# kuwt/model_matching

Measured on AMD Instinct MI355X. Metric: candidate poses verified/sec, higher is better.
Workload: dtype f32; 1 GPU; Cm: synthetic 20000-pt scene vs 5000-pt model, 65536 candidate transforms per step per GPU, eps=5mm; scene_points=20000, model_points=5000

## Files before the change

### model_matching_amd/csrc/lcp.hip

```cpp
#include <stdlib.h>
#include <string.h>

#include <cstring>


#include <algorithm>
#include <utility>

#include "kdtree.h"
#include "normal_cone.h"
#include "octant_lists.h"
#include "prims.h"
#include "stocs_ctx.h"

namespace stocs {

struct LcpArgs {
    const float4* mpos;
    const float4* mnrm;
    const int32_t* mperm;
    int M;
    const int32_t* top;
    const uint4* cells;
    const uint4* flat;
    const float4* list;
    const float4* snrmw;
    const int32_t* cand_trial;
    size_t snrmw_stride;
    const float* chunk_r;
    float ox, oy, oz, inv_h, inv_h4, h;
    int nx, ny, nz, nbx, nby;
    float sq_eps, dot_lo, eps;
    float bound_margin;
    int has_nearest;
    const int32_t* order;
    int xcd_blocks;
    unsigned long long* best;
    uint32_t id_offset;
    const float4* patch;
    const float4* sub;
    const float* dist;
    float gox, goy, goz, g, inv_g, cap;
    int gnx, gny, gnz;
#ifdef STOCS_TOOLS_BUILD
    int ablate;
#endif
};
#ifdef STOCS_TOOLS_BUILD
#define STOCS_ABLATE(a, bit) (((a).ablate & (bit)) != 0)
#else
#define STOCS_ABLATE(a, bit) false
#endif

__device__ __forceinline__ int lcp_candidate(const LcpArgs& a, int n, int w, int wpb = 4) {
    int blk = blockIdx.x;
    if (a.xcd_blocks == 1) {
        const int nb = gridDim.x, per = nb >> 3, rem = nb & 7, xcd = blk & 7;
        blk = xcd * per + (xcd < rem ? xcd : rem) + (blk >> 3);
    } else if (a.xcd_blocks > 1) {
        const int C = a.xcd_blocks, nb = gridDim.x, full = (nb / (8 * C)) * (8 * C);
        if (blk < full) {
            const int xcd = blk & 7, j = blk >> 3;
            blk = ((j / C) * 8 + xcd) * C + (j % C);
        }
    }
    const int slot = __builtin_amdgcn_readfirstlane(blk * wpb + w);
    if (slot >= n) return -1;
    return a.order ? __builtin_amdgcn_readfirstlane(a.order[slot]) : slot;
}


__device__ __forceinline__ const float4* lcp_weights_of(const LcpArgs& a, int cand) {
    if (!a.cand_trial) return a.snrmw;
    const int t = __builtin_amdgcn_readfirstlane(a.cand_trial[cand < 0 ? 0 : cand]);
    return (const float4*)((const char*)a.snrmw + (size_t)t * a.snrmw_stride);
}

#define DPP_QUAD_XOR1 0xB1
#define DPP_QUAD_XOR2 0x4E
#define DPP_HALF_MIRROR 0x141

__device__ __forceinline__ void lcp_add(unsigned long long& acc, float w) {
    if (w > 0.0f) acc += (unsigned long long)(w * 4294967296.0f);
}
__device__ __forceinline__ unsigned long long lcp_wave_sum(unsigned long long acc) {
    for (int off = 32; off > 0; off >>= 1) acc += __shfl_xor(acc, off, 64);
    return acc;
}
__device__ __forceinline__ float lcp_finish(unsigned long long total, int M) {
    return (float)((double)total * (1.0 / 4294967296.0) / (double)M);
}
__device__ __forceinline__ void lcp_store(const LcpArgs& a, float* __restrict__ out, int cand, unsigned long long total) {
    const float s = lcp_finish(total, a.M);
    out[cand] = s;
    if (a.best && s > 0.0f)
        atomicMax(a.best, best_key(s, a.id_offset + (uint32_t)cand));
}

template <bool IDX>
__device__ __forceinline__ void take_if_better(float d, int ei, float& gd, int& gi) {
    if (IDX) { if (d <= gd) { gd = d; gi = ei; } }
    else { if (d < gd || (d == gd && ei > gi)) { gd = d; gi = ei; } }
}

template <bool DETAIL, bool IDX = true>
__global__ __launch_bounds__(256) void lcp_kernel(LcpArgs a, const float* __restrict__ T16, float* __restrict__ out,
                                                  int n, int32_t* __restrict__ hit_out, uint8_t* __restrict__ cnt_out) {
    const int lane = threadIdx.x & 63;
    const int cand = lcp_candidate(a, n, threadIdx.x >> 6);
    if (cand < 0) return;
    const float* T = T16 + (size_t)cand * 16;
    const float4* __restrict__ snrmw = lcp_weights_of(a, cand);
    const float t0 = T[0], t1 = T[1], t2 = T[2], t4 = T[4], t5 = T[5], t6 = T[6], t8 = T[8], t9 = T[9], t10 = T[10],
                t12 = T[12], t13 = T[13], t14 = T[14];
    unsigned long long acc = 0ull;
    for (int i = lane; i < a.M; i += 64) {
        const float4 p = a.mpos[i];
        const float qx = ((t0 * p.x + t4 * p.y) + t8 * p.z) + t12;
        const float qy = ((t1 * p.x + t5 * p.y) + t9 * p.z) + t13;
        const float qz = ((t2 * p.x + t6 * p.y) + t10 * p.z) + t14;
        const float fx = floorf((qx - a.ox) * a.inv_h);
        const float fy = floorf((qy - a.oy) * a.inv_h);
        const float fz = floorf((qz - a.oz) * a.inv_h);
        int best = -1;
        if (fx >= 0.0f && fy >= 0.0f && fz >= 0.0f && fx < (float)a.nx && fy < (float)a.ny && fz < (float)a.nz) {
            const int cx = (int)fx, cy = (int)fy, cz = (int)fz;
            const int brick = a.top[((cz >> 3) * a.nby + (cy >> 3)) * a.nbx + (cx >> 3)];
            if (brick >= 0) {
                const uint4 cw = a.cells[(size_t)brick * 512 + (((cz & 7) << 6) | ((cy & 7) << 3) | (cx & 7))];
                float bd = a.sq_eps;
                const uint32_t cn = cw.y & STOCS_CONE_COUNT_MASK;
                for (uint32_t k = 0; k < cn; ++k) {
                    const float4 s = a.list[cw.x + k];
                    const float dx = qx - s.x, dy = qy - s.y, dz = qz - s.z;
                    const float d = dx * dx + (dy * dy + dz * dz);
                    take_if_better<IDX>(d, __float_as_int(s.w), bd, best);
                }
            }
        }
        bool counted = false;
        if (best >= 0) {
            const float4 nm = a.mnrm[i];
            const float nx = t0 * nm.x + (t4 * nm.y + t8 * nm.z);
            const float ny = t1 * nm.x + (t5 * nm.y + t9 * nm.z);
            const float nz = t2 * nm.x + (t6 * nm.y + t10 * nm.z);
            const float4 sn = snrmw[best];
            const float d = sn.x * nx + (sn.y * ny + sn.z * nz);
            counted = (d >= a.dot_lo) && (d <= 1.0f);
            if (counted) lcp_add(acc, sn.w);
        }
        if (DETAIL) {
            const int orig = a.mperm[i];
            hit_out[(size_t)cand * a.M + orig] = best;
            cnt_out[(size_t)cand * a.M + orig] = counted ? 1 : 0;
        }
    }
    acc = lcp_wave_sum(acc);
    if (lane == 0) lcp_store(a, out, cand, acc);
}

template <int CTRL>
__device__ __forceinline__ float dpp_f32(float v) {
    return __int_as_float(__builtin_amdgcn_update_dpp(0, __float_as_int(v), CTRL, 0xF, 0xF, true));
}
template <int CTRL>
__device__ __forceinline__ int dpp_i32(int v) {
    return __builtin_amdgcn_update_dpp(0, v, CTRL, 0xF, 0xF, true);
}

template <int GL>
__device__ __forceinline__ float group_min_nonneg(float v) {
    uint32_t u = __float_as_uint(v);
    if (GL >= 2) u = min(u, (uint32_t)__builtin_amdgcn_update_dpp((int)u, (int)u, DPP_QUAD_XOR1, 0xF, 0xF, false));
    if (GL >= 4) u = min(u, (uint32_t)__builtin_amdgcn_update_dpp((int)u, (int)u, DPP_QUAD_XOR2, 0xF, 0xF, false));
    if (GL == 8) u = min(u, (uint32_t)__builtin_amdgcn_update_dpp((int)u, (int)u, DPP_HALF_MIRROR, 0xF, 0xF, false));
    return __uint_as_float(u);
}

constexpr int lcp_waves_per_block(bool detail, bool split) { return (split || detail) ? 4 : 1; }

template <bool DETAIL, bool SPLIT>
__global__ __launch_bounds__(64 * lcp_waves_per_block(DETAIL, SPLIT)) void lcp_coop_kernel(LcpArgs a, const float* __restrict__ T16, float* __restrict__ out,
                                                       int n, int32_t* __restrict__ hit_out, uint8_t* __restrict__ cnt_out) {
    static_assert(!(DETAIL && SPLIT), "the detail form is not split");
    constexpr int WPB = lcp_waves_per_block(DETAIL, SPLIT);
    constexpr int UNR = 2;
    __shared__ float4 qt[WPB][64];
    __shared__ uint32_t qn[WPB][64];
    __shared__ uint32_t hl[WPB][64];
    __shared__ float rd[WPB][64];
    __shared__ int ri[WPB][64];
    __shared__ float qd[WPB][64];
    __shared__ unsigned long long part[WPB];
    const int lane = threadIdx.x & 63;
    const int sub = lane & 7, grp = lane >> 3;
    const int w = threadIdx.x >> 6;
    const int cand = SPLIT ? lcp_candidate(a, n, 0, 1) : lcp_candidate(a, n, w, WPB);
    if (cand < 0) return;
    const int first = SPLIT ? 64 * w : 0, stride = SPLIT ? 64 * WPB : 64;
    const float4* __restrict__ snrmw = lcp_weights_of(a, cand);
    const float* T = T16 + (size_t)cand * 16;
    const float t0 = T[0], t1 = T[1], t2 = T[2], t4 = T[4], t5 = T[5], t6 = T[6], t8 = T[8], t9 = T[9], t10 = T[10],
                t12 = T[12], t13 = T[13], t14 = T[14];
    unsigned long long acc = 0ull;
    for (int base = first; base < a.M; base += stride) {
        const int i = base + lane;
        float qx = 0.f, qy = 0.f, qz = 0.f, qcd = 0.f;
        uint32_t off = 0, cnt = 0;
        if (i < a.M) {
            const float4 p = a.mpos[i];
            qx = ((t0 * p.x + t4 * p.y) + t8 * p.z) + t12;
            qy = ((t1 * p.x + t5 * p.y) + t9 * p.z) + t13;
            qz = ((t2 * p.x + t6 * p.y) + t10 * p.z) + t14;
            const float ux = (qx - a.ox) * a.inv_h, uy = (qy - a.oy) * a.inv_h, uz = (qz - a.oz) * a.inv_h;
            const float fx = floorf(ux), fy = floorf(uy), fz = floorf(uz);
            if (fx >= 0.0f && fy >= 0.0f && fz >= 0.0f && fx < (float)a.nx && fy < (float)a.ny && fz < (float)a.nz) {
                const int cx = (int)fx, cy = (int)fy, cz = (int)fz;
                const int brick = STOCS_ABLATE(a, 1) ? -1 : a.top[((cz >> 3) * a.nby + (cy >> 3)) * a.nbx + (cx >> 3)];
                if (brick >= 0) {
                    uint4 cw = make_uint4(0u, 0u, 0u, 0u);
                    if (!STOCS_ABLATE(a, 128)) cw = a.cells[(size_t)brick * 512 + (((cz & 7) << 6) | ((cy & 7) << 3) | (cx & 7))];
                    const int sb = ((int)((uz - fz) * 4.0f) << 4) | ((int)((uy - fy) * 4.0f) << 2) | (int)((ux - fx) * 4.0f);
                    const uint32_t mw = a.has_nearest ? 0xFFFFFFFFu : (sb < 32 ? cw.z : cw.w);
                    off = cw.x; cnt = ((mw >> (sb & 31)) & 1u) ? (cw.y & STOCS_CONE_COUNT_MASK) : 0u;
                    if (STOCS_ABLATE(a, 2)) cnt = cw.x == 0xFFFFFFF1u ? 1u : 0u;
                    const float ex = qx - (a.ox + ((float)cx + 0.5f) * a.h), ey = qy - (a.oy + ((float)cy + 0.5f) * a.h),
                                ez = qz - (a.oz + ((float)cz + 0.5f) * a.h);
                    qcd = sqrtf(ex * ex + (ey * ey + ez * ez));
                }
            }
        }
        const bool hit = cnt != 0;
        const unsigned long long mask = __ballot(hit);
        int best = -1;
        if (mask) {
            const int nh = __popcll(mask);
            if (hit) {
                const int rank = __popcll(mask & ((1ull << lane) - 1ull));
                hl[w][rank] = (uint32_t)lane;
                qt[w][lane] = make_float4(qx, qy, qz, __int_as_float((int)off));
                qn[w][lane] = cnt;
                qd[w][lane] = qcd;
            }
            __builtin_amdgcn_wave_barrier();
            for (int s = 0; s < nh; s += 8) {
                const int slot = s + grp;
                const bool gact = slot < nh;
                const uint32_t L = gact ? hl[w][slot] : 0u;
                const float4 qq = qt[w][L];
                const uint32_t c = gact ? qn[w][L] : 0u;
                const float4* lp = a.list + (uint32_t)__float_as_int(qq.w) + sub;
                float gd = a.sq_eps;
                int gi = -1;
                const float qcg = qd[w][L];
                const uint32_t chunk0 = (uint32_t)__float_as_int(qq.w) >> 3;
                uint32_t nchunks = (c + 7u) >> 3;
                float gb = a.sq_eps;
                if (STOCS_ABLATE(a, 4)) nchunks = min(nchunks, (uint32_t)UNR);
                for (uint32_t j = 0; __any(j < nchunks); j += UNR) {
                    if (j < nchunks && j > 0 && (STOCS_ABLATE(a, 256) ? 0.0f : a.chunk_r[chunk0 + j]) - qcg > sqrtf(gb) + a.bound_margin) nchunks = 0;
                    float4 e[UNR];
#pragma unroll
                    for (int u = 0; u < UNR; ++u) {
                        e[u] = make_float4(1e30f, 1e30f, 1e30f, __int_as_float(-1));
                        if (j + u < nchunks) e[u] = lp[(j + u) << 3];
                    }
#pragma unroll
                    for (int u = 0; u < UNR; ++u) {
                        const float dx = qq.x - e[u].x, dy = qq.y - e[u].y, dz = qq.z - e[u].z;
                        const float d = dx * dx + (dy * dy + dz * dz);
                        const int ei = __float_as_int(e[u].w);
                        if (d < gd || (d == gd && ei > gi)) { gd = d; gi = ei; }
                    }
                    gb = fminf(gd, dpp_f32<DPP_QUAD_XOR1>(gd));
                    gb = fminf(gb, dpp_f32<DPP_QUAD_XOR2>(gb));
                    gb = fminf(gb, dpp_f32<DPP_HALF_MIRROR>(gb));
                }
                float dm = fminf(gd, dpp_f32<DPP_QUAD_XOR1>(gd));
                dm = fminf(dm, dpp_f32<DPP_QUAD_XOR2>(dm));
                dm = fminf(dm, dpp_f32<DPP_HALF_MIRROR>(dm));
                int im = (gd == dm) ? gi : -1;
                im = max(im, dpp_i32<DPP_QUAD_XOR1>(im));
                im = max(im, dpp_i32<DPP_QUAD_XOR2>(im));
                im = max(im, dpp_i32<DPP_HALF_MIRROR>(im));
                if (gact && sub == 0) { rd[w][L] = dm; ri[w][L] = im; }
            }
            __builtin_amdgcn_wave_barrier();
            if (hit) best = ri[w][lane];
            __builtin_amdgcn_wave_barrier();
        }
        bool counted = false;
        if (best >= 0 && STOCS_ABLATE(a, 8)) lcp_add(acc, 0.5f);
        else if (best >= 0) {
            const float4 nm = a.mnrm[i];
            const float nx = t0 * nm.x + (t4 * nm.y + t8 * nm.z);
            const float ny = t1 * nm.x + (t5 * nm.y + t9 * nm.z);
            const float nz = t2 * nm.x + (t6 * nm.y + t10 * nm.z);
            const float4 sn = snrmw[best];
            const float d = sn.x * nx + (sn.y * ny + sn.z * nz);
            counted = (d >= a.dot_lo) && (d <= 1.0f);
            if (counted) lcp_add(acc, sn.w);
        }
        if (DETAIL && i < a.M) {
            const int orig = a.mperm[i];
            hit_out[(size_t)cand * a.M + orig] = best;
            cnt_out[(size_t)cand * a.M + orig] = counted ? 1 : 0;
        }
    }
    acc = lcp_wave_sum(acc);
    if (SPLIT) {
        if (lane == 0) part[w] = acc;
        __syncthreads();
        if (threadIdx.x == 0) {
            unsigned long long total = 0;
#pragma unroll
            for (int k = 0; k < WPB; ++k) total += part[k];
            lcp_store(a, out, cand, total);
        }
    } else if (lane == 0) lcp_store(a, out, cand, acc);
}

__device__ __forceinline__ bool lcp_patch_dead(const LcpArgs& a, const float4 sp, float sn, float t0, float t1, float t2, float t4, float t5, float t6,
                                               float t8, float t9, float t10, float t12, float t13, float t14) {
    const float cx = ((t0 * sp.x + t4 * sp.y) + t8 * sp.z) + t12;
    const float cy = ((t1 * sp.x + t5 * sp.y) + t9 * sp.z) + t13;
    const float cz = ((t2 * sp.x + t6 * sp.y) + t10 * sp.z) + t14;
    const float mag = fabsf(cx) + (fabsf(cy) + fabsf(cz));
    if (!(mag < 1.0e18f)) return false;
    const float need = (sn * sp.w + a.eps * 1.002f) + (4.0e-6f + 4.0e-6f * mag);
    const float ux = (cx - a.gox) * a.inv_g, uy = (cy - a.goy) * a.inv_g, uz = (cz - a.goz) * a.inv_g;
    const float fx = floorf(ux), fy = floorf(uy), fz = floorf(uz);
    if (fx >= 1.0f && fy >= 1.0f && fz >= 1.0f && fx < (float)(a.gnx - 1) && fy < (float)(a.gny - 1) && fz < (float)(a.gnz - 1)) {
        const float v = a.dist[((uint32_t)(int)fz * (uint32_t)a.gny + (uint32_t)(int)fy) * (uint32_t)a.gnx + (uint32_t)(int)fx];
        const float ex = cx - (a.gox + (fx + 0.5f) * a.g), ey = cy - (a.goy + (fy + 0.5f) * a.g), ez = cz - (a.goz + (fz + 0.5f) * a.g);
        return v - sqrtf(ex * ex + (ey * ey + ez * ez)) > need;
    }
    return a.cap > need;
}

constexpr int LCP_SHARED_LIVE = 512;

constexpr bool lcp_queue_form_legal(bool detail, bool dense, bool split, bool flat, bool near, int cu, bool shared, bool gate) {
    return !(gate && (detail || dense || (split && cu == 16 && !shared))) && (cu == 16 || cu == 64) && (!shared || (split && cu == 16)) && (detail ? (!split && !flat && !(dense && near)) : (!dense || (split && !flat && !near)));
}

template <bool DETAIL, bool DENSE, bool SPLIT, bool FLAT, bool NEAR, int CU, bool SHARED, bool GATE>
__global__ __launch_bounds__(64 * lcp_waves_per_block(DETAIL, SPLIT), 8) void lcp_coopq_kernel(LcpArgs a, const float* __restrict__ T16, float* __restrict__ out,
                                                        int n, int32_t* __restrict__ hit_out, uint8_t* __restrict__ cnt_out) {
    static_assert(lcp_queue_form_legal(DETAIL, DENSE, SPLIT, FLAT, NEAR, CU, SHARED, GATE), "not one of the forms in the table above");
    constexpr int WPB = lcp_waves_per_block(DETAIL, SPLIT);
    constexpr bool IDX = !DENSE;
    constexpr bool EARLY = DENSE;
    constexpr int GL = 4, EPL = 8 / GL, NG = 64 / GL;
    constexpr int FIRST = DENSE ? 1 : 2, E0 = EPL * FIRST;
    constexpr bool NOSENT = !DENSE;
    constexpr int UNR = 1;
    constexpr int PIPE = 1;
    static_assert(!EARLY || (FIRST == 1 && !NOSENT), "early exit decides line by line");
    __shared__ float4 qt[WPB][128];
    __shared__ float qcd[EARLY ? WPB : 1][EARLY ? 128 : 1];
    __shared__ uint32_t qn[WPB][128];
    __shared__ uint32_t qs[WPB][128];
    __shared__ int ri[WPB][128];
    __shared__ uint8_t ord[WPB][64];
    __shared__ unsigned long long part[WPB];
    const int lane = threadIdx.x & 63;
    const int w = threadIdx.x >> 6;
    const int cand = SPLIT ? lcp_candidate(a, n, 0, 1) : lcp_candidate(a, n, w, WPB);
    if (cand < 0) return;
    const float4* __restrict__ snrmw = lcp_weights_of(a, cand);
    const float* T = T16 + (size_t)cand * 16;
    const float t0 = T[0], t1 = T[1], t2 = T[2], t4 = T[4], t5 = T[5], t6 = T[6], t8 = T[8], t9 = T[9], t10 = T[10],
                t12 = T[12], t13 = T[13], t14 = T[14];
    unsigned long long acc = 0ull;
    int head = 0, tail = 0;
    const float gnorm = GATE ? linear_norm_bound(t0, t1, t2, t4, t5, t6, t8, t9, t10) : 0.0f;
    const float gthr = GATE ? model_normal_gate_threshold(a.dot_lo, gnorm) : 0.0f;

    auto process = [&](int nq) {
        {
            uint32_t cls = 4;
            if (lane < nq) {
                const uint32_t nch = (qn[w][(head + lane) & 127] + 7u) >> 3;
                cls = nch <= (uint32_t)FIRST ? 1u : (nch <= (uint32_t)(FIRST + UNR) ? 2u : 3u);
            }
            const unsigned long long below = (1ull << lane) - 1ull;
            const unsigned long long m1 = __ballot(cls == 1u), m2 = __ballot(cls == 2u), m3 = __ballot(cls == 3u);
            const int n1 = __popcll(m1), n2 = __popcll(m2);
            const int pos = cls == 1u ? __popcll(m1 & below) : (cls == 2u ? n1 + __popcll(m2 & below) : n1 + n2 + __popcll(m3 & below));
            if (lane < nq) ord[w][pos] = (uint8_t)lane;
            __builtin_amdgcn_wave_barrier();
        }
        for (int s0 = 0; s0 < nq; s0 += NG * PIPE) {
            const int sub = lane & (GL - 1), grp = lane / GL;
            float4 e0[PIPE][E0];
            bool wide[PIPE];
            int idxs[PIPE];
            uint32_t cs[PIPE];
#pragma unroll
            for (int u = 0; u < PIPE; ++u) {
                const int slot = s0 + NG * u + grp;
                const bool gact = slot < nq;
                idxs[u] = (head + (int)ord[w][gact ? slot : 0]) & 127;
                cs[u] = gact ? qn[w][idxs[u]] : 0u;
                wide[u] = true;
                if (!NOSENT) {
#pragma unroll
                    for (int e = 0; e < E0; ++e) e0[u][e] = make_float4(1e30f, 1e30f, 1e30f, __int_as_float(-1));
                }
                if (STOCS_ABLATE(a, 4)) {
                    if (cs[u]) { const float4 qq0 = qt[w][idxs[u]]; e0[u][0] = make_float4(qq0.x, qq0.y, qq0.z, __int_as_float(0)); }
                    cs[u] = cs[u] ? 1u : 0u;
                }
                else if (NOSENT) {
                    const float4* l0 = a.list + (cs[u] ? (uint32_t)__float_as_int(qt[w][idxs[u]].w) : 0u) + sub;
                    const uint32_t last = cs[u] ? ((cs[u] - 1u) & ~7u) : 0u;
#pragma unroll
                    for (int e = 0; e < EPL; ++e) e0[u][e] = l0[GL * e];
                    wide[u] = FIRST > 1 && __any(cs[u] > 8u);
                    if (wide[u]) {
#pragma unroll
                        for (int e = EPL; e < E0; ++e) e0[u][e] = l0[min((uint32_t)(8 * (e / EPL)), last) + GL * (e % EPL)];
                    }
                }
                else if (cs[u]) {
                    const float4* l0 = a.list + (uint32_t)__float_as_int(qt[w][idxs[u]].w) + sub;
#pragma unroll
                    for (int e = 0; e < E0; ++e) e0[u][e] = l0[GL * e];
                }
            }
#pragma unroll
            for (int u = 0; u < PIPE; ++u) {
                const float4 qq = qt[w][idxs[u]];
                const uint32_t c = cs[u];
                const float4* lp = a.list + (uint32_t)__float_as_int(qq.w) + sub;
                const uint32_t last_line = c ? ((c - 1u) & ~7u) : 0u;
                float gd = a.sq_eps;
                int gi = -1;
#pragma unroll
                for (int e = 0; e < EPL; ++e) {
                    const float dx = qq.x - e0[u][e].x, dy = qq.y - e0[u][e].y, dz = qq.z - e0[u][e].z;
                    const float d = dx * dx + (dy * dy + dz * dz);
                    take_if_better<IDX>(d, __float_as_int(e0[u][e].w), gd, gi);
                }
                if (FIRST > 1 && wide[u]) {
#pragma unroll
                    for (int e = EPL; e < E0; ++e) {
                        const float dx = qq.x - e0[u][e].x, dy = qq.y - e0[u][e].y, dz = qq.z - e0[u][e].z;
                        const float d = dx * dx + (dy * dy + dz * dz);
                        take_if_better<IDX>(d, __float_as_int(e0[u][e].w), gd, gi);
                    }
                }
                if (EARLY) {
                    const float qcg = qcd[w][idxs[u]];
                    const uint32_t chunk0 = (uint32_t)__float_as_int(qq.w) >> 3;
                    uint32_t cc = c;
                    for (uint32_t k = 8; __any(k < cc); k += 8 * UNR) {
                        if (k < cc && a.chunk_r[chunk0 + (k >> 3)] - qcg > sqrtf(group_min_nonneg<GL>(gd)) + a.bound_margin) cc = 0;
                        float4 e[EPL];
                        if (k < cc) {
#pragma unroll
                            for (int x = 0; x < EPL; ++x) e[x] = lp[k + GL * x];
                        } else {
#pragma unroll
                            for (int x = 0; x < EPL; ++x) e[x] = make_float4(1e30f, 1e30f, 1e30f, __int_as_float(-1));
                        }
#pragma unroll
                        for (int x = 0; x < EPL; ++x) {
                            const float dx = qq.x - e[x].x, dy = qq.y - e[x].y, dz = qq.z - e[x].z;
                            const float d = dx * dx + (dy * dy + dz * dz);
                            take_if_better<IDX>(d, __float_as_int(e[x].w), gd, gi);
                        }
                    }
                } else {
                    for (uint32_t k = 8 * FIRST; __any(k < c); k += 8 * UNR) {
                        const uint32_t kk = min(k, last_line);
                        float4 e[EPL];
#pragma unroll
                        for (int x = 0; x < EPL; ++x) e[x] = lp[kk + GL * x];
#pragma unroll
                        for (int x = 0; x < EPL; ++x) {
                            const float dx = qq.x - e[x].x, dy = qq.y - e[x].y, dz = qq.z - e[x].z;
                            const float d = dx * dx + (dy * dy + dz * dz);
                            take_if_better<IDX>(d, __float_as_int(e[x].w), gd, gi);
                        }
                    }
                }
                const float dm = group_min_nonneg<GL>(gd);
                int im = (gd == dm) ? gi : -1;
                im = max(im, dpp_i32<DPP_QUAD_XOR1>(im));
                im = max(im, dpp_i32<DPP_QUAD_XOR2>(im));
                if (c && sub == 0) ri[w][idxs[u]] = im;
            }
        }
        __builtin_amdgcn_wave_barrier();
        if (lane < nq) {
            const int idx = (head + lane) & 127;
            const int best = ri[w][idx];
            const uint32_t slot_i = qs[w][idx];
            bool counted = false;
            if (best >= 0 && STOCS_ABLATE(a, 8)) { lcp_add(acc, 0.5f); }
            else if (best >= 0) {
                const float4 nm = STOCS_ABLATE(a, 16) ? make_float4(0.f, 0.f, 1.f, 0.f) : a.mnrm[slot_i];
                const float nx = t0 * nm.x + (t4 * nm.y + t8 * nm.z);
                const float ny = t1 * nm.x + (t5 * nm.y + t9 * nm.z);
                const float nz = t2 * nm.x + (t6 * nm.y + t10 * nm.z);
                const float4 sn = STOCS_ABLATE(a, 32) ? make_float4(nx, ny, nz, 0.5f) : snrmw[best];
                const float d = sn.x * nx + (sn.y * ny + sn.z * nz);
                counted = (d >= a.dot_lo) && (d <= 1.0f);
                if (counted) lcp_add(acc, sn.w);
            }
            if (DETAIL) {
                const int orig = a.mperm[slot_i];
                hit_out[(size_t)cand * a.M + orig] = best;
                cnt_out[(size_t)cand * a.M + orig] = counted ? 1 : 0;
            }
        }
        __builtin_amdgcn_wave_barrier();
    };

    auto step = [&](const int i, const float4 p) {
        float qx = 0.f, qy = 0.f, qz = 0.f, qcentre = 0.f, nearest = 0.f;
        uint32_t off = 0, cnt = 0, yw = 0;
        constexpr uint32_t cmask = STOCS_CONE_COUNT_MASK;
        if (!DETAIL || i < a.M) {
            qx = ((t0 * p.x + t4 * p.y) + t8 * p.z) + t12;
            qy = ((t1 * p.x + t5 * p.y) + t9 * p.z) + t13;
            qz = ((t2 * p.x + t6 * p.y) + t10 * p.z) + t14;
            const int c4x = __float2int_rd((qx - a.ox) * a.inv_h4), c4y = __float2int_rd((qy - a.oy) * a.inv_h4),
                      c4z = __float2int_rd((qz - a.oz) * a.inv_h4);
            const int cx = c4x >> 2, cy = c4y >> 2, cz = c4z >> 2;
            if ((unsigned)cx < (unsigned)a.nx && (unsigned)cy < (unsigned)a.ny && (unsigned)cz < (unsigned)a.nz) {
                const int sb = ((c4z & 3) << 4) | ((c4y & 3) << 2) | (c4x & 3);
                if (FLAT) {
                    uint4 cw = make_uint4(0u, 0u, 0u, 0u);
                    if (!STOCS_ABLATE(a, 1))
                        cw = a.flat[(uint32_t)((cz * a.ny + cy) * a.nx + cx)];
                    const uint32_t mw = sb < 32 ? cw.z : cw.w;
                    off = octant_word_flagged(cw.x) ? octant_line_offset(cw.x, (uint32_t)sb) : cw.x;
                    yw = cw.y; cnt = ((mw >> (sb & 31)) & 1u) ? (cw.y & cmask) : 0u;
                    if (STOCS_ABLATE(a, 2)) cnt = cw.x == 0xFFFFFFF1u ? 1u : 0u;
                } else {
                    const int brick = a.top[((cz >> 3) * a.nby + (cy >> 3)) * a.nbx + (cx >> 3)];
                    if (brick >= 0) {
                        const uint4 cw = a.cells[(uint32_t)brick * 512u + (uint32_t)(((cz & 7) << 6) | ((cy & 7) << 3) | (cx & 7))];
                        yw = cw.y;
                        if ((EARLY || NEAR) && a.has_nearest) { off = cw.x; cnt = cw.y & cmask; nearest = __uint_as_float(cw.z); }
                        else { const uint32_t mw = a.has_nearest ? 0xFFFFFFFFu : (sb < 32 ? cw.z : cw.w); off = cw.x; cnt = ((mw >> (sb & 31)) & 1u) ? (cw.y & cmask) : 0u; }
                    }
                }
            }
            if ((EARLY || (NEAR && a.has_nearest)) && cnt) {
                const float ex = qx - (a.ox + ((float)cx + 0.5f) * a.h), ey = qy - (a.oy + ((float)cy + 0.5f) * a.h), ez = qz - (a.oz + ((float)cz + 0.5f) * a.h);
                qcentre = sqrtf(ex * ex + (ey * ey + ez * ez));
                if (a.has_nearest && nearest - qcentre > a.eps + a.bound_margin) cnt = 0;
            }
            if (GATE && cnt && cone_rules_out_packed(yw, __float_as_uint(p.w), t0, t1, t2, t4, t5, t6, t8, t9, t10, gthr)) cnt = 0;
            if (DETAIL && cnt == 0) {
                const int orig = a.mperm[i];
                hit_out[(size_t)cand * a.M + orig] = -1;
                cnt_out[(size_t)cand * a.M + orig] = 0;
            }
        }
        const bool hit = cnt != 0;
        const unsigned long long mask = __ballot(hit);
        if (mask) {
            if (hit) {
                const int rank = __popcll(mask & ((1ull << lane) - 1ull));
                const int sl = (tail + rank) & 127;
                qt[w][sl] = make_float4(qx, qy, qz, __int_as_float((int)off));
                qn[w][sl] = cnt;
                qs[w][sl] = (uint32_t)i;
                if (EARLY) qcd[w][sl] = qcentre;
            }
            tail += __popcll(mask);
            __builtin_amdgcn_wave_barrier();
            if (tail - head >= 64) {
                process(64);
                head += 64;
            }
        }
    };
    if (CU == 16) {
    __shared__ uint16_t live_q[WPB][128];
    const int nsteps = (a.M + 63) >> 6;
    if (SHARED) {
    __shared__ int live_n;
    uint16_t* const live_all = &live_q[0][0];
    static_assert(!SHARED || WPB * 128 == LCP_SHARED_LIVE, "the shared list is the memory of the per-wave rings");
    if (threadIdx.x == 0) live_n = 0;
    const int nsubs = (a.M + 15) >> 4;
    const float snorm = GATE ? gnorm : (a.patch ? linear_norm_bound(t0, t1, t2, t4, t5, t6, t8, t9, t10) : 0.0f);
    unsigned long long lm[2];
#pragma unroll
    for (int j = 0; j < 2; ++j) {
        const int q = ((w + 4 * j) << 6) + lane;
        bool live = q < nsubs;
        if (a.patch && live && !STOCS_ABLATE(a, 64))
            live = !lcp_patch_dead(a, a.sub[q], snorm, t0, t1, t2, t4, t5, t6, t8, t9, t10, t12, t13, t14);
        lm[j] = __ballot(live);
    }
    __syncthreads();
#pragma unroll
    for (int j = 0; j < 2; ++j) {
        if (lm[j]) {
            int base = 0;
            if (lane == 0) base = atomicAdd(&live_n, __popcll(lm[j]));
            base = __builtin_amdgcn_readfirstlane(base);
            if ((lm[j] >> lane) & 1ull)
                live_all[base + __popcll(lm[j] & ((1ull << lane) - 1ull))] = (uint16_t)(((w + 4 * j) << 6) + lane);
        }
    }
    __syncthreads();
    const int nlive = __builtin_amdgcn_readfirstlane(live_n);
    const int nst = (nlive + 3) >> 2;
    const int mine = __builtin_amdgcn_readfirstlane((nst + 3 - w) >> 2);
    const int e0 = 4 * w + (lane >> 4);
    auto slot = [&](int k) { const int e = e0 + 16 * k; return e < nlive ? ((int)live_all[e] << 4) + (lane & 15) : (nsteps << 6) + lane; };
    if (mine > 0) {
        int i = slot(0);
        float4 p_next = a.mpos[i];
        for (int k = 0; k < mine; ++k) {
            const int ic = i;
            const float4 p = p_next;
            i = k + 1 < mine ? slot(k + 1) : ic;
            p_next = a.mpos[i];
            step(ic, p);
        }
    }
    } else {
    const int wfirst = SPLIT ? w : 0, nw = SPLIT ? WPB : 1;
    const int nsub = __builtin_amdgcn_readfirstlane(4 * ((nsteps - wfirst + nw - 1) / nw));
    const float snorm = GATE ? gnorm : (a.patch ? linear_norm_bound(t0, t1, t2, t4, t5, t6, t8, t9, t10) : 0.0f);
    int qh = 0, qtl = 0;
    for (int s0 = 0;; s0 += 64) {
        {
            const int kl = s0 + lane, q = 4 * (wfirst + (kl >> 2) * nw) + (kl & 3);
            const bool in = kl < nsub && (q << 4) < a.M;
            bool live = in;
            if (a.patch && live && !STOCS_ABLATE(a, 64))
                live = !lcp_patch_dead(a, a.sub[q], snorm, t0, t1, t2, t4, t5, t6, t8, t9, t10, t12, t13, t14);
            const unsigned long long mask = __ballot(live);
            if (live) live_q[w][(qtl + __popcll(mask & ((1ull << lane) - 1ull))) & 127] = (uint16_t)q;
            qtl += __popcll(mask);
            if (DETAIL && a.patch) {
                unsigned long long dead = __ballot(in && !live);
                while (dead) {
                    const int j = __builtin_ctzll(dead);
                    dead &= dead - 1ull;
                    const int id = ((4 * (wfirst + ((s0 + j) >> 2) * nw) + ((s0 + j) & 3)) << 4) + lane;
                    if (lane < 16 && id < a.M) {
                        const int orig = a.mperm[id];
                        hit_out[(size_t)cand * a.M + orig] = -1;
                        cnt_out[(size_t)cand * a.M + orig] = 0;
                    }
                }
            }
            __builtin_amdgcn_wave_barrier();
        }
        const bool last = s0 + 64 >= nsub;
        const int g = lane >> 4;
        auto slot = [&](int t) { return g < t ? ((int)live_q[w][(qh + g) & 127] << 4) + (lane & 15) : (nsteps << 6) + lane; };
        int t = min(qtl - qh, 4);
        if (t == 4 || (last && t > 0)) {
            int i = slot(t);
            float4 p_next = a.mpos[i];
            for (;;) {
                const int ic = i;
                const float4 p = p_next;
                qh += t;
                t = min(qtl - qh, 4);
                const bool more = t == 4 || (last && t > 0);
                i = more ? slot(t) : ic;
                p_next = a.mpos[i];
                step(ic, p);
                if (!more) break;
            }
        }
        if (last) break;
    }
    }
    } else {
    const int nsteps = (a.M + 63) >> 6;
    const int wfirst = SPLIT ? w : 0, nw = SPLIT ? WPB : 1;
    const int nk = (nsteps - wfirst + nw - 1) / nw;
    const float snorm = GATE ? gnorm : (a.patch ? linear_norm_bound(t0, t1, t2, t4, t5, t6, t8, t9, t10) : 0.0f);
    for (int k0 = 0; k0 < nk; k0 += 64) {
        const int kk = k0 + lane;
        bool live = kk < nk;
        if (a.patch && live && !STOCS_ABLATE(a, 64))
            live = !lcp_patch_dead(a, a.patch[wfirst + kk * nw], snorm, t0, t1, t2, t4, t5, t6, t8, t9, t10, t12, t13, t14);
        unsigned long long todo = __ballot(live);
        if (DETAIL && a.patch) {
            unsigned long long dead = __ballot(kk < nk && !live);
            while (dead) {
                const int j = __builtin_ctzll(dead);
                dead &= dead - 1ull;
                const int i = ((wfirst + (k0 + j) * nw) << 6) + lane;
                if (i < a.M) {
                    const int orig = a.mperm[i];
                    hit_out[(size_t)cand * a.M + orig] = -1;
                    cnt_out[(size_t)cand * a.M + orig] = 0;
                }
            }
        }
        if (!todo) continue;
        int j = __builtin_ctzll(todo);
        float4 p_next = a.mpos[((wfirst + (k0 + j) * nw) << 6) + lane];
        for (;;) {
            const int i = ((wfirst + (k0 + j) * nw) << 6) + lane;
            const float4 p = p_next;
            todo &= todo - 1ull;
            j = todo ? __builtin_ctzll(todo) : j;
            p_next = a.mpos[((wfirst + (k0 + j) * nw) << 6) + lane];
            step(i, p);
            if (!todo) break;
        }
    }
    }
    if (tail - head > 0) process(tail - head);
    acc = lcp_wave_sum(acc);
    if (SPLIT) {
        if (lane == 0) part[w] = acc;
        __syncthreads();
        if (threadIdx.x == 0) {
            unsigned long long total = 0;
#pragma unroll
            for (int k = 0; k < WPB; ++k) total += part[k];
            lcp_store(a, out, cand, total);
        }
    } else if (lane == 0) lcp_store(a, out, cand, acc);
}

template <bool DETAIL>
__global__ __launch_bounds__(256) void lcp_exact_kernel(LcpArgs a, const float* __restrict__ T16, float* __restrict__ out, int n,
                                                        int32_t* __restrict__ hit_out, uint8_t* __restrict__ cnt_out,
                                                        const KdNodeP* __restrict__ kd_nodes, const float4* __restrict__ kd_pts,
                                                        unsigned long long* __restrict__ ties) {
    const int lane = threadIdx.x & 63;
    const int cand = lcp_candidate(a, n, threadIdx.x >> 6);
    if (cand < 0) return;
    const float* T = T16 + (size_t)cand * 16;
    const float4* __restrict__ snrmw = lcp_weights_of(a, cand);
    const float t0 = T[0], t1 = T[1], t2 = T[2], t4 = T[4], t5 = T[5], t6 = T[6], t8 = T[8], t9 = T[9], t10 = T[10],
                t12 = T[12], t13 = T[13], t14 = T[14];
    unsigned long long acc = 0ull, n_flag = 0ull, n_changed = 0ull;
    for (int i = lane; i < a.M; i += 64) {
        const float4 p = a.mpos[i];
        const float qx = ((t0 * p.x + t4 * p.y) + t8 * p.z) + t12;
        const float qy = ((t1 * p.x + t5 * p.y) + t9 * p.z) + t13;
        const float qz = ((t2 * p.x + t6 * p.y) + t10 * p.z) + t14;
        const float fx = floorf((qx - a.ox) * a.inv_h);
        const float fy = floorf((qy - a.oy) * a.inv_h);
        const float fz = floorf((qz - a.oz) * a.inv_h);
        int best = -1;
        bool tie = false;
        float bd = a.sq_eps;
        if (fx >= 0.0f && fy >= 0.0f && fz >= 0.0f && fx < (float)a.nx && fy < (float)a.ny && fz < (float)a.nz) {
            const int cx = (int)fx, cy = (int)fy, cz = (int)fz;
            const int brick = a.top[((cz >> 3) * a.nby + (cy >> 3)) * a.nbx + (cx >> 3)];
            if (brick >= 0) {
                const uint4 cw = a.cells[(size_t)brick * 512 + (((cz & 7) << 6) | ((cy & 7) << 3) | (cx & 7))];
                const uint32_t cn = cw.y & STOCS_CONE_COUNT_MASK;
                for (uint32_t k = 0; k < cn; ++k) {
                    const float4 s = a.list[cw.x + k];
                    const float dx = qx - s.x, dy = qy - s.y, dz = qz - s.z;
                    const float d = dx * dx + (dy * dy + dz * dz);
                    const int ei = __float_as_int(s.w);
                    if (d < bd) { bd = d; best = ei; tie = false; }
                    else if (d == bd) { if (best >= 0) { tie = true; best = max(best, ei); } else best = ei; }
                }
            }
        }
        if (tie || (best >= 0 && bd == a.sq_eps)) {
            const int kb = kd_query_closest(kd_nodes, kd_pts, qx, qy, qz, a.sq_eps);
            n_flag++;
            if (kb != best) n_changed++;
            best = kb;
        }
        bool counted = false;
        if (best >= 0) {
            const float4 nm = a.mnrm[i];
            const float nx = t0 * nm.x + (t4 * nm.y + t8 * nm.z);
            const float ny = t1 * nm.x + (t5 * nm.y + t9 * nm.z);
            const float nz = t2 * nm.x + (t6 * nm.y + t10 * nm.z);
            const float4 sn = snrmw[best];
            const float d = sn.x * nx + (sn.y * ny + sn.z * nz);
            counted = (d >= a.dot_lo) && (d <= 1.0f);
            if (counted) lcp_add(acc, sn.w);
        }
        if (DETAIL) {
            const int orig = a.mperm[i];
            hit_out[(size_t)cand * a.M + orig] = best;
            cnt_out[(size_t)cand * a.M + orig] = counted ? 1 : 0;
        }
    }
    acc = lcp_wave_sum(acc);
    n_flag = lcp_wave_sum(n_flag);
    n_changed = lcp_wave_sum(n_changed);
    if (lane == 0) {
        lcp_store(a, out, cand, acc);
        if (n_flag) atomicAdd(&ties[0], n_flag);
        if (n_changed) atomicAdd(&ties[1], n_changed);
    }
}

__global__ __launch_bounds__(256) void best_kernel(const float* __restrict__ lcp, int n, uint32_t id_offset, unsigned long long* __restrict__ best) {
    unsigned long long k = 0;
    for (int i = blockIdx.x * blockDim.x + threadIdx.x; i < n; i += gridDim.x * blockDim.x) {
        const float s = lcp[i];
        if (s > 0.0f) { const unsigned long long key = best_key(s, id_offset + (uint32_t)i); k = key > k ? key : k; }
    }
    k = wave_max_key(k);
    if ((threadIdx.x & 63) == 0 && k) atomicMax(best, k);
}

__global__ __launch_bounds__(1024) void best_single_kernel(const float* __restrict__ lcp, int n, uint32_t id_offset, unsigned long long* __restrict__ best) {
    __shared__ unsigned long long sh[16];
    unsigned long long k = 0;
    for (int i = threadIdx.x; i < n; i += 1024) {
        const float s = lcp[i];
        if (s > 0.0f) {
            const unsigned long long key = ((unsigned long long)__float_as_uint(s) << 32) | (unsigned long long)(0xFFFFFFFFu - (id_offset + (uint32_t)i));
            k = key > k ? key : k;
        }
    }
    for (int off = 32; off > 0; off >>= 1) {
        const unsigned long long o = __shfl_xor(k, off, 64);
        k = o > k ? o : k;
    }
    if ((threadIdx.x & 63) == 0) sh[threadIdx.x >> 6] = k;
    __syncthreads();
    if (threadIdx.x == 0) {
        for (int w = 1; w < 16; ++w) k = sh[w] > k ? sh[w] : k;
        *best = k;
    }
}

__device__ __forceinline__ uint32_t spread10(uint32_t x) {
    x &= 0x3ff; x = (x | (x << 16)) & 0x30000ff; x = (x | (x << 8)) & 0x300f00f; x = (x | (x << 4)) & 0x30c30c3; x = (x | (x << 2)) & 0x9249249;
    return x;
}
__global__ __launch_bounds__(256) void order_keys_kernel(const float* __restrict__ T16, int n, float ox, float oy, float oz, float sx, float sy, float sz,
                                                         uint32_t* __restrict__ keys, int32_t* __restrict__ vals, unsigned long long* __restrict__ best) {
    const int i = blockIdx.x * blockDim.x + threadIdx.x;
    if (i == 0 && best) *best = 0ull;
    if (i >= n) return;
    const float* T = T16 + (size_t)i * 16;
    const float qx = fminf(fmaxf((T[12] - ox) * sx, 0.0f), 255.0f), qy = fminf(fmaxf((T[13] - oy) * sy, 0.0f), 255.0f),
                qz = fminf(fmaxf((T[14] - oz) * sz, 0.0f), 255.0f);
    keys[i] = (spread10((uint32_t)qz) << 2) | (spread10((uint32_t)qy) << 1) | spread10((uint32_t)qx);
    vals[i] = i;
}

enum LcpKernel { LCP_PLAIN, LCP_STEP, LCP_QUEUE, LCP_EXACT };
struct LcpForm {
    LcpKernel kernel;
    bool detail;
    bool dense;
    bool split;
    bool flat, near;
    int cu;
    bool shared;
    bool gate;
};

static bool lcp_variant_selectable(int v) { return v == 99 || v == 0 || v == 24 || v == 31 || v == 39; }

static LcpForm choose_lcp_form(const stocs_ctx* c, const LcpArgs& a, bool detail) {
    LcpForm f = {LCP_QUEUE, detail, false, false, false, false, 64, false, false};
    if (c->exact_ties) { f.kernel = LCP_EXACT; return f; }
    f.dense = c->grid.d_chunk_r != NULL;
    const int variant = c->lcp_variant >= 0 ? c->lcp_variant : 99;
    if (variant == 0) f.kernel = (detail && f.dense) ? LCP_STEP : LCP_PLAIN;
    else if (variant == 31 && f.dense) f.kernel = LCP_STEP;
    const bool split = c->lcp_split && a.M >= 512;
    if (f.kernel == LCP_STEP) f.split = !detail && split;
    if (f.kernel == LCP_QUEUE) {
        f.split = !detail && (f.dense || split);
        f.flat = !detail && !f.dense && c->lcp_flat && a.flat;
        f.near = !f.dense && a.has_nearest;
        f.cu = (a.patch && c->lcp_cull_unit == 16) ? 16 : 64;
        f.shared = f.split && f.cu == 16 && a.M <= 16 * LCP_SHARED_LIVE;
        f.gate = !detail && !f.dense && c->grid.has_cones && c->lcp_normal_gate != 0 && !(f.split && f.cu == 16 && !f.shared);
    }
    return f;
}

typedef void (*LcpScanFn)(LcpArgs, const float*, float*, int, int32_t*, uint8_t*);

template <int I>
static LcpScanFn lcp_queue_fn() {
    constexpr bool DETAIL = (I & 1) != 0, DENSE = (I & 2) != 0, SPLIT = (I & 4) != 0, FLAT = (I & 8) != 0, NEAR = (I & 16) != 0;
    constexpr int CU = (I & 32) ? 16 : 64;
    constexpr bool SHARED = (I & 64) != 0, GATE = (I & 128) != 0;
    if constexpr (lcp_queue_form_legal(DETAIL, DENSE, SPLIT, FLAT, NEAR, CU, SHARED, GATE)) return lcp_coopq_kernel<DETAIL, DENSE, SPLIT, FLAT, NEAR, CU, SHARED, GATE>;
    else return NULL;
}
template <int... I>
static LcpScanFn lcp_queue_fn(const LcpForm& f, std::integer_sequence<int, I...>) {
    static const LcpScanFn table[] = {lcp_queue_fn<I>()...};
    return table[(f.detail ? 1 : 0) | (f.dense ? 2 : 0) | (f.split ? 4 : 0) | (f.flat ? 8 : 0) | (f.near ? 16 : 0) | (f.cu == 16 ? 32 : 0) | (f.shared ? 64 : 0) | (f.gate ? 128 : 0)];
}
// ... 422 lines not shown
```

Measured before the change: 81.29 million poses/s.

## Prefetch patch records and chain queue records to shorten load latency in shared LCP path

In the shared-list kernel form, the patch sub-records are now loaded before the transform is read. The dead-patch test is split into a probe step, a batched distance-grid load for both halves, and a verdict step, so the memory loads can overlap. The queue processing packs each entry's list offset, length and ring index into a per-wave shared record array ordered by class, and prefetches the next record one trip ahead. This replaces several dependent shared-memory lookups per trip. The weight add becomes branchless. The cost is extra shared memory and registers, plus an unconditional dist read at cell 0 for probes that fall outside the grid.

```diff
diff --git a/model_matching_amd/csrc/lcp.hip b/model_matching_amd/csrc/lcp.hip
--- a/model_matching_amd/csrc/lcp.hip
+++ b/model_matching_amd/csrc/lcp.hip
@@ -80,6 +80,9 @@
 #define DPP_QUAD_XOR2 0x4E
 #define DPP_HALF_MIRROR 0x141
 
+__device__ __forceinline__ unsigned long long lcp_addend(float w) {
+    return w > 0.0f ? (unsigned long long)(w * 4294967296.0f) : 0ull;
+}
 __device__ __forceinline__ void lcp_add(unsigned long long& acc, float w) {
     if (w > 0.0f) acc += (unsigned long long)(w * 4294967296.0f);
 }
@@ -320,6 +323,31 @@
     } else if (lane == 0) lcp_store(a, out, cand, acc);
 }
 
+struct LcpPatchProbe {
+    float cx, cy, cz, fx, fy, fz;
+    uint32_t cell;
+    bool inside;
+};
+__device__ __forceinline__ LcpPatchProbe lcp_patch_probe(const LcpArgs& a, const float4 sp, float t0, float t1, float t2, float t4, float t5, float t6,
+                                                         float t8, float t9, float t10, float t12, float t13, float t14) {
+    LcpPatchProbe p;
+    p.cx = ((t0 * sp.x + t4 * sp.y) + t8 * sp.z) + t12;
+    p.cy = ((t1 * sp.x + t5 * sp.y) + t9 * sp.z) + t13;
+    p.cz = ((t2 * sp.x + t6 * sp.y) + t10 * sp.z) + t14;
+    const float mag = fabsf(p.cx) + (fabsf(p.cy) + fabsf(p.cz));
+    const float ux = (p.cx - a.gox) * a.inv_g, uy = (p.cy - a.goy) * a.inv_g, uz = (p.cz - a.goz) * a.inv_g;
+    p.fx = floorf(ux); p.fy = floorf(uy); p.fz = floorf(uz);
+    p.inside = (mag < 1.0e18f) && p.fx >= 1.0f && p.fy >= 1.0f && p.fz >= 1.0f && p.fx < (float)(a.gnx - 1) && p.fy < (float)(a.gny - 1) && p.fz < (float)(a.gnz - 1);
+    p.cell = p.inside ? ((uint32_t)(int)p.fz * (uint32_t)a.gny + (uint32_t)(int)p.fy) * (uint32_t)a.gnx + (uint32_t)(int)p.fx : 0u;
+    return p;
+}
+__device__ __forceinline__ bool lcp_patch_verdict(const LcpArgs& a, const LcpPatchProbe& p, float radius, float sn, float v) {
+    const float mag = fabsf(p.cx) + (fabsf(p.cy) + fabsf(p.cz));
+    const float need = (sn * radius + a.eps * 1.002f) + (4.0e-6f + 4.0e-6f * mag);
+    const float ex = p.cx - (a.gox + (p.fx + 0.5f) * a.g), ey = p.cy - (a.goy + (p.fy + 0.5f) * a.g), ez = p.cz - (a.goz + (p.fz + 0.5f) * a.g);
+    const float room = p.inside ? v - sqrtf(ex * ex + (ey * ey + ez * ez)) : a.cap;
+    return (mag < 1.0e18f) && room > need;
+}
 __device__ __forceinline__ bool lcp_patch_dead(const LcpArgs& a, const float4 sp, float sn, float t0, float t1, float t2, float t4, float t5, float t6,
                                                float t8, float t9, float t10, float t12, float t13, float t14) {
     const float cx = ((t0 * sp.x + t4 * sp.y) + t8 * sp.z) + t12;
@@ -356,6 +384,7 @@
     constexpr bool NOSENT = !DENSE;
     constexpr int UNR = 1;
     constexpr int PIPE = 1;
+    constexpr bool CHAIN = SHARED;
     static_assert(!EARLY || (FIRST == 1 && !NOSENT), "early exit decides line by line");
     __shared__ float4 qt[WPB][128];
     __shared__ float qcd[EARLY ? WPB : 1][EARLY ? 128 : 1];
@@ -363,12 +392,20 @@
     __shared__ uint32_t qs[WPB][128];
     __shared__ int ri[WPB][128];
     __shared__ uint8_t ord[WPB][64];
+    __shared__ uint2 srec[CHAIN ? WPB : 1][CHAIN ? 64 : 1];
     __shared__ unsigned long long part[WPB];
     const int lane = threadIdx.x & 63;
     const int w = threadIdx.x >> 6;
     const int cand = SPLIT ? lcp_candidate(a, n, 0, 1) : lcp_candidate(a, n, w, WPB);
     if (cand < 0) return;
     const float4* __restrict__ snrmw = lcp_weights_of(a, cand);
+    const bool patch_on = SHARED && !STOCS_ABLATE(a, 64);
+    float4 wsp[2] = {make_float4(0.f, 0.f, 0.f, 0.f), make_float4(0.f, 0.f, 0.f, 0.f)};
+    if (SHARED) {
+        const int last_sub = max(((a.M + 15) >> 4) - 1, 0);
+#pragma unroll
+        for (int j = 0; j < 2; ++j) wsp[j] = a.sub[min((int)(((threadIdx.x >> 6) + 4 * j) << 6) + lane, last_sub)];
+    }
     const float* T = T16 + (size_t)cand * 16;
     const float t0 = T[0], t1 = T[1], t2 = T[2], t4 = T[4], t5 = T[5], t6 = T[6], t8 = T[8], t9 = T[9], t10 = T[10],
                 t12 = T[12], t13 = T[13], t14 = T[14];
@@ -380,19 +417,28 @@
     auto process = [&](int nq) {
         {
             uint32_t cls = 4;
+            uint2 rec = make_uint2(0u, 0u);
             if (lane < nq) {
-                const uint32_t nch = (qn[w][(head + lane) & 127] + 7u) >> 3;
+                const int idx = (head + lane) & 127;
+                const uint32_t len = qn[w][idx];
+                const uint32_t nch = (len + 7u) >> 3;
                 cls = nch <= (uint32_t)FIRST ? 1u : (nch <= (uint32_t)(FIRST + UNR) ? 2u : 3u);
+                if (CHAIN) rec = make_uint2((uint32_t)__float_as_int(qt[w][idx].w), len | ((uint32_t)idx << 16));
             }
             const unsigned long long below = (1ull << lane) - 1ull;
             const unsigned long long m1 = __ballot(cls == 1u), m2 = __ballot(cls == 2u), m3 = __ballot(cls == 3u);
             const int n1 = __popcll(m1), n2 = __popcll(m2);
             const int pos = cls == 1u ? __popcll(m1 & below) : (cls == 2u ? n1 + __popcll(m2 & below) : n1 + n2 + __popcll(m3 & below));
-            if (lane < nq) ord[w][pos] = (uint8_t)lane;
+            if (CHAIN) { if (lane < nq) srec[w][pos] = rec; }
+            else if (lane < nq) ord[w][pos] = (uint8_t)lane;
             __builtin_amdgcn_wave_barrier();
         }
+        static_assert(!CHAIN || PIPE == 1, "one record per trip");
+        uint2 rec_next = make_uint2(0u, 0u);
+        if (CHAIN) rec_next = srec[w][lane / GL];
         for (int s0 = 0; s0 < nq; s0 += NG * PIPE) {
             const int sub = lane & (GL - 1), grp = lane / GL;
+            const uint2 rec = s0 + grp < nq ? rec_next : make_uint2(0u, (uint32_t)(head & 127) << 16);
             float4 e0[PIPE][E0];
             bool wide[PIPE];
             int idxs[PIPE];
@@ -401,8 +447,8 @@
             for (int u = 0; u < PIPE; ++u) {
                 const int slot = s0 + NG * u + grp;
                 const bool gact = slot < nq;
-                idxs[u] = (head + (int)ord[w][gact ? slot : 0]) & 127;
-                cs[u] = gact ? qn[w][idxs[u]] : 0u;
+                idxs[u] = CHAIN ? (int)((rec.y >> 16) & 127u) : (head + (int)ord[w][gact ? slot : 0]) & 127;
+                cs[u] = gact ? (CHAIN ? (rec.y & 0xFFFFu) : qn[w][idxs[u]]) : 0u;
                 wide[u] = true;
                 if (!NOSENT) {
 #pragma unroll
@@ -413,7 +459,7 @@
                     cs[u] = cs[u] ? 1u : 0u;
                 }
                 else if (NOSENT) {
-                    const float4* l0 = a.list + (cs[u] ? (uint32_t)__float_as_int(qt[w][idxs[u]].w) : 0u) + sub;
+                    const float4* l0 = a.list + (cs[u] ? (CHAIN ? rec.x : (uint32_t)__float_as_int(qt[w][idxs[u]].w)) : 0u) + sub;
                     const uint32_t last = cs[u] ? ((cs[u] - 1u) & ~7u) : 0u;
 #pragma unroll
                     for (int e = 0; e < EPL; ++e) e0[u][e] = l0[GL * e];
@@ -424,11 +470,12 @@
                     }
                 }
                 else if (cs[u]) {
-                    const float4* l0 = a.list + (uint32_t)__float_as_int(qt[w][idxs[u]].w) + sub;
+                    const float4* l0 = a.list + (CHAIN ? rec.x : (uint32_t)__float_as_int(qt[w][idxs[u]].w)) + sub;
 #pragma unroll
                     for (int e = 0; e < E0; ++e) e0[u][e] = l0[GL * e];
                 }
             }
+            if (CHAIN) rec_next = srec[w][min(s0 + NG * PIPE, 64 - NG * PIPE) + grp];
 #pragma unroll
             for (int u = 0; u < PIPE; ++u) {
                 const float4 qq = qt[w][idxs[u]];
@@ -506,9 +553,11 @@
                 const float ny = t1 * nm.x + (t5 * nm.y + t9 * nm.z);
                 const float nz = t2 * nm.x + (t6 * nm.y + t10 * nm.z);
                 const float4 sn = STOCS_ABLATE(a, 32) ? make_float4(nx, ny, nz, 0.5f) : snrmw[best];
+                const unsigned long long add = CHAIN ? lcp_addend(sn.w) : 0ull;
                 const float d = sn.x * nx + (sn.y * ny + sn.z * nz);
                 counted = (d >= a.dot_lo) && (d <= 1.0f);
-                if (counted) lcp_add(acc, sn.w);
+                if (CHAIN) acc += counted ? add : 0ull;
+                else if (counted) lcp_add(acc, sn.w);
             }
             if (DETAIL) {
                 const int orig = a.mperm[slot_i];
@@ -592,13 +641,22 @@
     const int nsubs = (a.M + 15) >> 4;
     const float snorm = GATE ? gnorm : (a.patch ? linear_norm_bound(t0, t1, t2, t4, t5, t6, t8, t9, t10) : 0.0f);
     unsigned long long lm[2];
-#pragma unroll
-    for (int j = 0; j < 2; ++j) {
-        const int q = ((w + 4 * j) << 6) + lane;
-        bool live = q < nsubs;
-        if (a.patch && live && !STOCS_ABLATE(a, 64))
-            live = !lcp_patch_dead(a, a.sub[q], snorm, t0, t1, t2, t4, t5, t6, t8, t9, t10, t12, t13, t14);
-        lm[j] = __ballot(live);
+    {
+        bool live[2];
+        LcpPatchProbe pp[2];
+        float fv[2] = {0.f, 0.f};
+#pragma unroll
+        for (int j = 0; j < 2; ++j) live[j] = ((w + 4 * j) << 6) + lane < nsubs;
+        if (patch_on) {
+#pragma unroll
+            for (int j = 0; j < 2; ++j) pp[j] = lcp_patch_probe(a, wsp[j], t0, t1, t2, t4, t5, t6, t8, t9, t10, t12, t13, t14);
+#pragma unroll
+            for (int j = 0; j < 2; ++j) fv[j] = a.dist[pp[j].cell];
+#pragma unroll
+            for (int j = 0; j < 2; ++j) live[j] = live[j] && !lcp_patch_verdict(a, pp[j], wsp[j].w, snorm, fv[j]);
+        }
+#pragma unroll
+        for (int j = 0; j < 2; ++j) lm[j] = __ballot(live[j]);
     }
     __syncthreads();
 #pragma unroll
```

New measurement: 83.66 million poses/s, median of 6. 1.03x the previous value.
